# jewettaij/visfd

Measured on AMD Instinct MI355X. Metric: Mvoxels/s (Gauss+DoG+TV pipeline) on 1024^3 float32; % HBM roofline, higher is better.
Workload: dtype f32

## Files before the change

visfd_amd/build.py:

```python
import concurrent.futures
import os
import subprocess
import sys
import time

HERE = os.path.dirname(os.path.abspath(__file__))
ROOT = os.path.dirname(HERE)
CSRC = os.path.join(HERE, "csrc")
OBJDIR = os.path.join(ROOT, "build", "visfd_hip")
LIB = os.path.join(HERE, "libvisfd_hip.so")

SOURCES = ["host_math.cpp", "blob_post.cpp", "connect.cpp", "watershed_host.cpp", "context.hip", "api.hip", "blob_job.hip", "gauss.hip", "blob.hip", "select.hip", "tv.hip", "resample.hip", "slab.hip", "morph.hip", "morph_levels.hip", "extrema.hip", "filter3d.hip", "draw.hip", "watershed.hip", "median.hip", "intensity.hip", "distance.hip", "find_spheres.hip", "discard_overlap.hip", "connect_seeds.hip", "connect_graph_host.cpp", "connect_graph.hip", "voxelize.hip", "surface_points.hip", "close_surface.hip"]
TV_VARIANT = [("tv_tiled.hip", "tv_tiled", ["-fno-slp-vectorize"]), ("tv_box.hip", "tv_box", ["-fno-slp-vectorize"]),
              ("tv_list.hip", "tv_list", ["-fno-slp-vectorize"]),
              ("ridge.hip", "ridge", [])]
PAIR_FLAGS = ["-fno-slp-vectorize"]
VARIANTS = TV_VARIANT + [("gauss_pair.hip", "gauss_pair", PAIR_FLAGS)] + [("gauss_fused.hip", "gauss_fused_h%d" % h, ["-DVH_FUSED_H=%d" % h, "-fno-slp-vectorize"])
                         for h in range(1, 9)]
HEADERS = ["common.hpp", "exact_div.hpp", "tv_common.hpp", "select_pick.hpp", "eigen3.hpp", "union_find.hpp", "tile.hpp", "watershed_host.hpp", "intensity.hpp", "connect_host.hpp", "connect_graph.hpp", os.path.join("..", "..", "include", "visfd_hip.h")]

HIPCC = os.environ.get("HIPCC", "/opt/rocm/bin/hipcc")
FLAGS = ["--offload-arch=gfx950", "-O3", "-std=c++17", "-fPIC", "-ffp-contract=off", "-fno-fast-math",
         "-Wall", "-Wno-unused-function"]


def _mtime(p):
    return os.path.getmtime(p) if os.path.exists(p) else 0.0


def _compile(src, obj, extra=()):
    t0 = time.time()
    cmd = [HIPCC] + FLAGS + list(extra) + ["-x", "hip", "-c", os.path.join(CSRC, src), "-o", obj]
    r = subprocess.run(cmd, capture_output=True, text=True)
    return src, r.returncode, r.stdout + r.stderr, time.time() - t0


def build(force=False, jobs=4, verbose=True):
    os.makedirs(OBJDIR, exist_ok=True)
    newest_header = max(_mtime(os.path.join(CSRC, h)) for h in HEADERS)
    todo, objs = [], []
    units = [(s, os.path.splitext(s)[0], []) for s in SOURCES] + VARIANTS
    flagfile = os.path.join(OBJDIR, "flags.txt")
    flagsig = repr((FLAGS, VARIANTS))
    if not os.path.exists(flagfile) or open(flagfile).read() != flagsig:
        force = True
    for s, stem, extra in units:
        obj = os.path.join(OBJDIR, stem + ".o")
        objs.append(obj)
        if force or _mtime(obj) < max(_mtime(os.path.join(CSRC, s)), newest_header):
            todo.append((s, obj, extra))
    if todo:
        with concurrent.futures.ThreadPoolExecutor(max_workers=jobs) as ex:
            for (src, rc, out, dt), (_, obj, _e) in zip(ex.map(lambda a: _compile(*a), todo), todo):
                if verbose:
                    print("[visfd_amd.build] %-22s %5.1fs %s" % (os.path.basename(obj), dt, "ok" if rc == 0 else "FAILED"))
                if rc != 0:
                    sys.stderr.write(out)
                    raise RuntimeError("hipcc failed on " + src)
                elif out.strip() and verbose:
                    sys.stderr.write(out)
    with open(flagfile, "w") as f:
        f.write(flagsig)
    if todo or not os.path.exists(LIB) or _mtime(LIB) < max(_mtime(o) for o in objs):
        cmd = [HIPCC, "--offload-arch=gfx950", "-shared", "-fPIC", "-o", LIB] + objs
        r = subprocess.run(cmd, capture_output=True, text=True)
        if r.returncode != 0:
            sys.stderr.write(r.stdout + r.stderr)
            raise RuntimeError("link failed")
        if verbose:
            print("[visfd_amd.build] linked", LIB)
    build_cli(verbose)
    return LIB
# ... 28 lines not shown
```

visfd_amd/csrc/api.hip:

```cpp
#include <algorithm>
#include <cmath>
#include <vector>

#include "common.hpp"
#include "tv_common.hpp"

namespace vh {

int gauss_dev(visfd_hip_ctx* ctx, const float* src, float* dst, const float* mask, i64 nx, i64 ny, i64 nz,
              const float sigma[3], const int hw[3], bool normalize, const GaussOpts& o) {
  VH_REQUIRE(ctx && src && dst && sigma && hw, "null argument");
  std::vector<float> t[3];
  for (int d = 0; d < 3; d++) {
    VH_REQUIRE(sigma[d] >= 0.0f, "sigma must be non-negative");
    VH_REQUIRE(hw[d] >= 0 && hw[d] <= MAX_HALFWIDTH, "filter halfwidth must be in [0, 64]");
    t[d].resize(2 * hw[d] + 1);
    host_gauss_taps(sigma[d], hw[d], t[d].data());
  }
  return dev_separable3d(ctx, src, dst, mask, nx, ny, nz, t[0].data(), hw[0], t[1].data(), hw[1], t[2].data(), hw[2],
                         normalize, o);
}

static int log_pair_try(visfd_hip_ctx* ctx, const float* src, float* dst, i64 nx, i64 ny, i64 nz, const float sa[3],
                        const float sb[3], const int hw[3], float scale, float* A, float* B) {
// ... 520 lines not shown
                             float cutoff, int curves) {
  VH_REQUIRE(ctx && sal && dir && ten, "null argument");
  VH_HIP(hipSetDevice(ctx->device));
  VH_TRY(check_dims(nx, ny, nz));
  const Stage st = {ctx, (size_t)(nx * ny * nz)};
  float *dsal, *pdir, *pten, *aos6, *dms = nullptr, *dmd = nullptr;
  VH_TRY(st.up(WS_H2D_0, sal, &dsal));
  VH_TRY(st.up_planar(WS_H2D_1, WS_H2D_2, dir, 3, &pdir));
  VH_TRY(st.out(WS_H2D_3, &pten, 6));
  VH_TRY(st.up(WS_H2D_4, mask_src, &dms));
  if (mask_dst == mask_src) dmd = dms;
  else VH_TRY(st.up(WS_A, mask_dst, &dmd));
  VH_TRY(dev_tv_dense_stick(ctx, dsal, pdir, pten, dms, dmd, nx, ny, nz, 0, nz, sigma_tv, exponent, cutoff, curves != 0));
  VH_TRY(st.out(WS_B, &aos6, 6));
  return st.down_interleaved(ten, pten, aos6, 6, dmd, true);
}

int visfd_hip_tv_weight_sum(visfd_hip_ctx* ctx, const float* sal, float* den, const float* mask_src,
                            const float* mask_dst, int64_t nx, int64_t ny, int64_t nz, float sigma_tv, float cutoff) {
  VH_REQUIRE(ctx && sal && den, "null argument");
  VH_HIP(hipSetDevice(ctx->device));
  VH_TRY(check_dims(nx, ny, nz));
  const Stage st = {ctx, (size_t)(nx * ny * nz)};
  float *dsal, *dden, *dms = nullptr, *dmd = nullptr;
  VH_TRY(st.up(WS_H2D_0, sal, &dsal));
  VH_TRY(st.up(WS_H2D_1, den, &dden));
  VH_TRY(st.up(WS_H2D_4, mask_src, &dms));
  if (mask_dst == mask_src) dmd = dms;
  else VH_TRY(st.up(WS_A, mask_dst, &dmd));
  VH_TRY(dev_tv_weight_sum(ctx, dsal, dden, dms, dmd, nx, ny, nz, sigma_tv, cutoff));
  return st.down(den, dden);
}

static int membrane_queued(visfd_hip_ctx* ctx, i64 nx, i64 ny, i64 nz, float sigma, int order, float best_fraction, float sigma_tv,
                           int exponent, float cutoff, const float* smoothed, float* sal, float* ten, float* dir, bool zero_dir,
                           const float* peak_img, const float* peak_bg, float* thr_out) {
  hipStream_t st = ctx->stream;
  const i64 n = nx * ny * nz;
  VH_TRY(select_rank_check((uint64_t)n, best_fraction));
  if (!ctx->stage_pinned) VH_HIP(hipHostMalloc(&ctx->stage_pinned, sizeof(StageReadback)));
  if (!ctx->stage_event) VH_HIP(hipEventCreateWithFlags(&ctx->stage_event, hipEventDisableTiming));
  StageReadback* block = nullptr;
  VH_TRY(ws(ctx, WS_SELECT, 1, &block));
  VH_HIP(hipMemsetAsync(block, 0, sizeof(*block), st));
  VH_TRY(dev_select_queue(ctx, sal, nullptr, n, best_fraction, &block->sel));
  const float* const thr_dev = &block->sel.thr;
  TvStagePlan plan;
  VH_TRY(dev_tv_stage_count(ctx, sal, thr_dev, nullptr, nx, ny, nz, sigma_tv, exponent, cutoff, &block->list_total,
                            &block->list_flags, &plan));
  const StageReadback* const got = static_cast<const StageReadback*>(ctx->stage_pinned);
  VH_HIP(hipMemcpyAsync(ctx->stage_pinned, block, sizeof(*block), hipMemcpyDeviceToHost, st));
  VH_HIP(hipEventRecord(ctx->stage_event, st));
  if (zero_dir) VH_HIP(hipMemsetAsync(dir, 0, sizeof(float) * 3 * (size_t)n, st));
  VH_TRY(dev_ridge_directions(ctx, smoothed, sal, nx, ny, nz, sigma, order, dir, thr_dev));
  VH_HIP(hipEventSynchronize(ctx->stage_event));
  float thr = 0.0f;
  VH_TRY(select_result(got->sel, &thr));
  if (thr_out) *thr_out = thr;
  int rc = dev_tv_stage_vote(ctx, plan, got->list_total, got->list_flags, sal, dir, ten, nullptr, nx, ny, nz, exponent);
  if (rc == TV_DECLINED) {
    VH_TRY(dev_apply_threshold(ctx, sal, n, thr));
    rc = dev_tv_dense_stick(ctx, sal, dir, ten, nullptr, nullptr, nx, ny, nz, 0, nz, sigma_tv, exponent, cutoff, false);
  }
  VH_TRY(rc);
  return dev_tensor_saliency(ctx, ten, nullptr, n, order, sal, peak_img, peak_bg);
}

static int membrane_stage(visfd_hip_ctx* ctx, const float* src, const float* mask, i64 nx, i64 ny, i64 nz, float sigma, float ratio,
                          int order, float best_fraction, float threshold_abs, float sigma_tv, int exponent, float cutoff,
                          float sigma_background, int normalize_background, float* bg, float* smoothed, float* sal, float* ten,
                          float* dir, bool zero_dir, float* thr_out) {
  const i64 n = nx * ny * nz;
  if (sigma_background > 0.0f)
    VH_TRY(visfd_hip_peak_background_dev(ctx, src, mask, nx, ny, nz, sigma_background, ratio, normalize_background, bg));
  else bg = nullptr;
  VH_TRY(visfd_hip_ridge_scores_bg_dev(ctx, src, mask, nx, ny, nz, sigma, ratio, order, bg, sal, smoothed));
  if (ctx->opt.membrane_queue && sigma_tv > 0.0f && best_fraction >= 0.0f && !mask) {
    const int rc = membrane_queued(ctx, nx, ny, nz, sigma, order, best_fraction, sigma_tv, exponent, cutoff, smoothed, sal, ten, dir,
                                   zero_dir, bg ? src : nullptr, bg, thr_out);
    if (rc != TV_DECLINED) return rc;
  }
  float thr = threshold_abs;
  if (best_fraction >= 0.0f) VH_TRY(dev_threshold_fraction(ctx, sal, mask, n, best_fraction, &thr));
  else VH_TRY(dev_apply_threshold(ctx, sal, n, thr));
  if (thr_out) *thr_out = thr;
  if (zero_dir) VH_HIP(hipMemsetAsync(dir, 0, sizeof(float) * 3 * (size_t)n, ctx->stream));
  VH_TRY(dev_ridge_directions(ctx, smoothed, sal, nx, ny, nz, sigma, order, dir));
  if (sigma_tv > 0.0f) {
    VH_TRY(dev_tv_dense_stick(ctx, sal, dir, ten, mask, mask, nx, ny, nz, 0, nz, sigma_tv, exponent, cutoff, false));
    VH_TRY(dev_tensor_saliency(ctx, ten, mask, n, order, sal, bg ? src : nullptr, bg));
  }
  return VISFD_HIP_OK;
}

int visfd_hip_membrane_detect_bg_dev(visfd_hip_ctx* ctx, const float* src, const float* mask, int64_t nx,
                                     int64_t ny, int64_t nz, float sigma, float ratio, int order,
                                     float best_fraction, float threshold_abs, float sigma_tv, int exponent,
                                     float cutoff, float sigma_background, int normalize_background, float* sal, float* ten,
                                     float* dir, float* thr_out) {
  VH_REQUIRE(ctx && src && sal, "null argument");
  VH_REQUIRE(order == 0 || order == 1, "unsupported eigenvalue order");
  VH_REQUIRE(best_fraction <= 1.0f, "fraction must be <= 1");
  VH_HIP(hipSetDevice(ctx->device));
  VH_TRY(check_dims(nx, ny, nz));
  const i64 n = nx * ny * nz;
  float* d = dir;
  if (!d) VH_TRY(ws(ctx, WS_TVAUX, (size_t)(3 * n), &d));
  float *smoothed = nullptr, *bg = nullptr, *t = ten;
  VH_TRY(ws(ctx, WS_D, (size_t)n, &smoothed));
  if (sigma_background > 0.0f) VH_TRY(ws(ctx, WS_C, (size_t)n, &bg));
  if (!t && sigma_tv > 0.0f) VH_TRY(ws(ctx, WS_B, (size_t)(6 * n), &t));
  return membrane_stage(ctx, src, mask, nx, ny, nz, sigma, ratio, order, best_fraction, threshold_abs, sigma_tv, exponent, cutoff,
                        sigma_background, normalize_background, bg, smoothed, sal, t, d, dir != nullptr, thr_out);
// ... 242 lines not shown
```

visfd_amd/csrc/common.hpp:

```cpp
#pragma once

#include <hip/hip_runtime.h>

#include <cstdint>
#include <cstdio>
#include <cstring>
#include <string>
#include <vector>

#include "../../include/visfd_hip.h"

namespace vh {

typedef int64_t i64;

void set_error(const std::string& msg);
int fail(int code, const std::string& msg);

#define VH_HIP(expr)                                                                         \
  do {                                                                                       \
    hipError_t _e = (expr);                                                                  \
    if (_e != hipSuccess)                                                                    \
      return vh::fail(_e == hipErrorOutOfMemory ? VISFD_HIP_ENOMEM : VISFD_HIP_EDEVICE,      \
                      std::string(#expr) + ": " + hipGetErrorString(_e));                    \
// ... 35 lines not shown
  WS_F3D_TAB,
  WS_DRAW_OWNER,
  WS_DRAW_TAB,
  WS_WSH_KIND,
  WS_WSH_LINK,
  WS_WSH_C,
  WS_WSH_STATE,
  WS_WSH_SEEDS,
  WS_WSH_FLAGS,
  WS_MEDIAN_TAB,
  WS_INTENSITY,
  WS_DIST_DSQ,
  WS_DIST_STACK,
  WS_DIST_POINTS,
  WS_FS_RECORDS,
  WS_FS_QUERIES,
  WS_CG_WORD,
  WS_CG_AUX,
  WS_CG_LIST,
  WS_CG_REC,
  WS_CG_SEEDS,
  WS_CG_CLUSTER,
  WS_CG_COUNTERS,
  WS_CG_SETTLE,
  WS_CG_LINKS,
  WS_OVL_LIST,
  WS_OVL_CELLS,
  WS_OVL_TEMP,
  WS_VOX_TOGGLE,
  WS_VOX_MESH,
  WS_SP_BITS,
  WS_SP_CHUNKS,
  WS_SP_LIST,
  WS_SP_OUT,
  WS_SP_SCRATCH,
  WS_CS_ACC,
  WS_CS_GRID,
  WS_CS_AUX,
  WS_SELECT,
  WS_NSLOTS
};

struct BlobJob;

}

struct visfd_hip_options {
  int gauss_3pass = 0;
  int gauss_cfg = 0;
  int gauss_wg_per_cu = 2;
  int log_pair = 1;
  int log_pair_chunk = 0;
  int membrane_queue = 1;
  int tv_dense = 0;
  int tv_fma = 0;
  int gauss_fma = 0;
  int eig_f32 = 0;
  int tv_zrun = 0;
  int tv_no_replay = 0;
  int tv_exact_tiled = 0;
  int tv_no_fold = 0;
  int tv_poison = 0;
  int tv_reserve_wg = 0;
  int tv_max_wg = 0;
  int64_t blob_test_cap = 0;
  int morph_general = 0;
  int morph_levels = 1;
  int filter3d_general = 0;
  int median_general = 0;
  int distance_general = 0;
  int discard_overlap_host = 0;
  int discard_overlap_time = 0;
  int discard_overlap_max_rounds = 256;
  int find_spheres_host = 0;
  int watershed_host = 0;
  int stats_blocks = 0;
  int connect_time = 0;
  int connect_settle = 0;
  int draw_time = 0;
  int voxelize_bisect = 0;
  int voxelize_time = 0;
  int surface_steps_cap = 256;
  int surface_points_time = 0;
  int close_surface_rtol_exp = 5;
  int close_surface_max_cycles = 20;
  int close_surface_time = 0;
  int debug = 0;
};

struct visfd_hip_ctx {
  visfd_hip_options opt;
  int device = 0;
  hipStream_t stream = nullptr;
  bool own_stream = false;
  void* slot_ptr[vh::WS_NSLOTS] = {};
  size_t slot_bytes[vh::WS_NSLOTS] = {};
  std::vector<unsigned char> slot_key[vh::WS_NSLOTS];
  int num_cus = 256;
  hipStream_t aux_stream = nullptr;
  void* stage_pinned = nullptr;
  hipEvent_t stage_event = nullptr;
  int morph_last_path = -1;
  struct {
    int64_t n = 0, ncols = 0;
    float den = 0.0f;
  } f3d;
// ... 360 lines not shown
```

visfd_amd/csrc/context.hip:

```cpp
#include <cctype>
#include <cstdlib>

#include "common.hpp"

namespace vh {

static thread_local std::string g_last_error;
void set_error(const std::string& msg) { g_last_error = msg; }
int fail(int code, const std::string& msg) {
  g_last_error = msg;
  return code;
}

int ws_get(visfd_hip_ctx* ctx, Slot s, size_t bytes, void** out) {
  if (bytes == 0) bytes = 16;
  if (ctx->slot_bytes[s] < bytes) {
    ctx->slot_key[s].clear();
    if (ctx->slot_ptr[s] && (s == WS_CAND || s == WS_SCANCNT)) VH_TRY(blob_jobs_drain(ctx));
    if (ctx->slot_ptr[s]) {
      VH_HIP(hipStreamSynchronize(ctx->stream));
      VH_HIP(hipFree(ctx->slot_ptr[s]));
      ctx->slot_ptr[s] = nullptr;
      ctx->slot_bytes[s] = 0;
    }
    void* p = nullptr;
    hipError_t e = hipMalloc(&p, bytes);
    if (e != hipSuccess)
      return fail(VISFD_HIP_ENOMEM, "hipMalloc of " + std::to_string(bytes) + " bytes failed: " +
                                        hipGetErrorString(e));
    ctx->slot_ptr[s] = p;
    ctx->slot_bytes[s] = bytes;
  }
  *out = ctx->slot_ptr[s];
  return VISFD_HIP_OK;
}

bool ws_holds(const visfd_hip_ctx* ctx, Slot s, const void* key, size_t key_bytes) {
  const std::vector<unsigned char>& k = ctx->slot_key[s];
  return key_bytes > 0 && k.size() == key_bytes && std::memcmp(k.data(), key, key_bytes) == 0;
}

int ws_put(visfd_hip_ctx* ctx, Slot s, const void* key, size_t key_bytes, const void* host, size_t bytes) {
  ctx->slot_key[s].clear();
  VH_HIP(hipStreamSynchronize(ctx->stream));
  void* d = nullptr;
  VH_TRY(ws_get(ctx, s, bytes, &d));
  VH_HIP(hipMemcpyAsync(d, host, bytes, hipMemcpyHostToDevice, ctx->stream));
  VH_HIP(hipStreamSynchronize(ctx->stream));
  const unsigned char* k = static_cast<const unsigned char*>(key);
  ctx->slot_key[s].assign(k, k + key_bytes);
  return VISFD_HIP_OK;
}

namespace {

struct OptionDesc {
  const char* name;
  int visfd_hip_options::*i = nullptr;
  int64_t visfd_hip_options::*l = nullptr;
  OptionDesc(const char* n, int visfd_hip_options::*f) : name(n), i(f) {}
  OptionDesc(const char* n, int64_t visfd_hip_options::*f) : name(n), l(f) {}
};
#define VH_OPT(field) {#field, &visfd_hip_options::field}
const OptionDesc kOptions[] = {
    VH_OPT(gauss_3pass), VH_OPT(gauss_cfg), VH_OPT(gauss_wg_per_cu), VH_OPT(log_pair), VH_OPT(log_pair_chunk),
    VH_OPT(membrane_queue),
    VH_OPT(tv_dense), VH_OPT(tv_fma), VH_OPT(gauss_fma), VH_OPT(eig_f32), VH_OPT(tv_zrun), VH_OPT(tv_no_replay),
    VH_OPT(tv_exact_tiled), VH_OPT(tv_no_fold), VH_OPT(tv_poison), VH_OPT(tv_reserve_wg), VH_OPT(tv_max_wg),
    VH_OPT(blob_test_cap), VH_OPT(morph_general), VH_OPT(morph_levels), VH_OPT(filter3d_general), VH_OPT(median_general),
    VH_OPT(distance_general), VH_OPT(discard_overlap_host), VH_OPT(discard_overlap_time),
    VH_OPT(discard_overlap_max_rounds), VH_OPT(find_spheres_host), VH_OPT(watershed_host), VH_OPT(stats_blocks),
    VH_OPT(connect_time), VH_OPT(connect_settle), VH_OPT(draw_time), VH_OPT(voxelize_bisect), VH_OPT(voxelize_time),
    VH_OPT(surface_steps_cap), VH_OPT(surface_points_time), VH_OPT(close_surface_rtol_exp),
    VH_OPT(close_surface_max_cycles), VH_OPT(close_surface_time), VH_OPT(debug),
};
#undef VH_OPT
bool set_option(visfd_hip_options* o, const char* name, int64_t value) {
  for (const OptionDesc& d : kOptions) {
    if (std::strcmp(d.name, name) != 0) continue;
    if (d.i) o->*(d.i) = (int)value; else o->*(d.l) = value;
    return true;
  }
  return false;
}
bool get_option(const visfd_hip_options* o, const char* name, int64_t* value) {
  for (const OptionDesc& d : kOptions) {
    if (std::strcmp(d.name, name) != 0) continue;
    *value = d.i ? (int64_t)(o->*(d.i)) : o->*(d.l);
    return true;
  }
  return false;
}
void options_from_environment(visfd_hip_options* o) {
  for (const OptionDesc& d : kOptions) {
    std::string env = "VISFD_HIP_";
    for (const char* c = d.name; *c; c++) env += (char)std::toupper((unsigned char)*c);
    if (const char* e = std::getenv(env.c_str())) set_option(o, d.name, (int64_t)std::atoll(e));
  }
}

}
}

using namespace vh;

extern "C" {

int visfd_hip_abi_version(void) { return 10; }
const char* visfd_hip_last_error(void) { return g_last_error.c_str(); }

int visfd_hip_create(int device, void* stream, visfd_hip_ctx** out) {
  VH_REQUIRE(out, "null output pointer");
  int count = 0;
  hipError_t e = hipGetDeviceCount(&count);
  if (e != hipSuccess || count <= 0)
    return fail(VISFD_HIP_EDEVICE, "no HIP device available (libvisfd_hip has no CPU fallback)");
  VH_REQUIRE(device >= 0 && device < count, "bad device ordinal");
  VH_HIP(hipSetDevice(device));
  hipDeviceProp_t prop;
// ... 91 lines not shown
```

visfd_amd/csrc/ridge.hip:

```cpp
#include "common.hpp"
#include "eigen3.hpp"

namespace vh {

namespace {

constexpr int BLOCK = 256;

struct Stencil {
  const float* S;
  i64 c;
  i64 sx, sy, sz;
  __device__ __forceinline__ float at(int dx, int dy, int dz) const {
    return S[c + dx * sx + dy * sy + dz * sz];
  }
};

__device__ __forceinline__ void hessian_at(const Stencil& f, float s2, float h6[6]) {
  const float f0 = f.at(0, 0, 0);
  const float two_f0 = 2 * f0;
  const float hxx = (f.at(1, 0, 0) + f.at(-1, 0, 0)) - two_f0;
  const float hyy = (f.at(0, 1, 0) + f.at(0, -1, 0)) - two_f0;
  const float hzz = (f.at(0, 0, 1) + f.at(0, 0, -1)) - two_f0;
  const float hxy = 0.25f * (((f.at(1, 1, 0) + f.at(-1, -1, 0)) - f.at(1, -1, 0)) - f.at(-1, 1, 0));
  const float hyz = 0.25f * (((f.at(0, 1, 1) + f.at(0, -1, -1)) - f.at(0, 1, -1)) - f.at(0, -1, 1));
  const float hzx = 0.25f * (((f.at(1, 0, 1) + f.at(-1, 0, -1)) - f.at(-1, 0, 1)) - f.at(1, 0, -1));
  h6[0] = hxx * s2; h6[1] = hyy * s2; h6[2] = hzz * s2;
  h6[3] = hxy * s2; h6[4] = hyz * s2; h6[5] = hzx * s2;
}

__device__ __forceinline__ bool voxel_of_block(int nx, int ny, int& ix, int& iy, int& iz) {
  const int xblocks = (nx + BLOCK - 1) / BLOCK;
  unsigned b = blockIdx.x;
  const int bx = b % xblocks;
  b /= xblocks;
  iy = b % ny;
  iz = b / ny;
  ix = bx * BLOCK + threadIdx.x;
  return ix < nx;
}

__device__ __forceinline__ Stencil clamped_stencil(const float* S, int ix, int iy, int iz, int nx, int ny,
                                                   int nz) {
  const int x = min(max(ix, 1), nx - 2), y = min(max(iy, 1), ny - 2), z = min(max(iz, 1), nz - 2);
  Stencil f;
  f.S = S;
  f.sx = 1; f.sy = nx; f.sz = (i64)nx * ny;
  f.c = (i64)z * f.sz + (i64)y * nx + x;
  return f;
}

template <bool F32>
__device__ __forceinline__ void saliency_dir(const float h6[6], int order, float& sal, float dir[3]) {
  float d6[6];
  eig::diagonalize_flat<F32>(h6, order, d6);
  const double l1 = d6[0], l2 = d6[1];
  double N = l1 * l1 - l2 * l2;
  N *= N;
  sal = (float)N;
  eig::shoemake_row0(d6 + 3, dir);
}

__global__ void __launch_bounds__(BLOCK)
hessian_kernel(const float* __restrict__ S, const float* __restrict__ mask, int nx, int ny, int nz,
               float sigma, float* __restrict__ grad, float* __restrict__ hess) {
  int ix, iy, iz;
  if (!voxel_of_block(nx, ny, ix, iy, iz)) return;
  const i64 nvox = (i64)nx * ny * nz;
  const i64 v = ((i64)iz * ny + iy) * nx + ix;
  if (mask && mask[v] == 0.0f) return;
  const Stencil f = clamped_stencil(S, ix, iy, iz, nx, ny, nz);
  if (grad) {
    const float g0 = 0.5f * (f.at(1, 0, 0) - f.at(-1, 0, 0));
    const float g1 = 0.5f * (f.at(0, 1, 0) - f.at(0, -1, 0));
    const float g2 = 0.5f * (f.at(0, 0, 1) - f.at(0, 0, -1));
    grad[v] = g0 * sigma;
    grad[nvox + v] = g1 * sigma;
    grad[2 * nvox + v] = g2 * sigma;
  }
  if (hess) {
    float h6[6];
    hessian_at(f, sigma * sigma, h6);
#pragma unroll
    for (int c = 0; c < 6; c++) hess[c * nvox + v] = h6[c];
  }
}

template <bool F32>
__global__ void __launch_bounds__(BLOCK)
hessian_saliency_kernel(const float* __restrict__ hess, const float* __restrict__ mask, i64 nvox,
                        int order, float* __restrict__ sal, float* __restrict__ dir) {
  const i64 v = (i64)blockIdx.x * BLOCK + threadIdx.x;
  if (v >= nvox) return;
  if (mask && mask[v] == 0.0f) { sal[v] = 0.0f; return; }
  float h6[6];
#pragma unroll
  for (int c = 0; c < 6; c++) h6[c] = hess[c * nvox + v];
  float s, d[3];
  saliency_dir<F32>(h6, order, s, d);
  sal[v] = s;
  dir[v] = d[0];
  dir[nvox + v] = d[1];
  dir[2 * nvox + v] = d[2];
}

template <bool F32>
__global__ void __launch_bounds__(BLOCK)
ridge_fused_kernel(const float* __restrict__ S, const float* __restrict__ mask, int nx, int ny, int nz,
                   float sigma, int order, float* __restrict__ sal, float* __restrict__ dir) {
  int ix, iy, iz;
  if (!voxel_of_block(nx, ny, ix, iy, iz)) return;
  const i64 nvox = (i64)nx * ny * nz;
  const i64 v = ((i64)iz * ny + iy) * nx + ix;
// ... 263 lines not shown
```

visfd_amd/csrc/tv_common.hpp:

```cpp
#pragma once

#include <algorithm>

#include "common.hpp"

namespace vh {

constexpr int TV_DECLINED = -1;

inline int tv_padded_row(int h) {
  int sp = 2 * h + 1;
  while ((sp & 7) != 4) sp++;
  return sp;
}

inline int tv_box_row(int h) {
  int sp = 2 * h + 1 + 3;
  while ((sp & 7) != 4) sp++;
  return sp;
}
inline int tv_box_slice(int h) { return (2 * h + 1 + 6) * tv_box_row(h) + 8; }

struct TvTableLayout {
  size_t packed, padded, box_tol, box_exact, box_tol_sq;
// ... 31 lines not shown

inline int tv_plan_units(const visfd_hip_ctx* ctx, int default_zrun, int tiles_x, int tiles_y, i64 z_out0, i64 z_out1,
                         int* zrun, i64* nblk) {
  int zr = default_zrun;
  if (ctx->opt.tv_zrun >= 1 && ctx->opt.tv_zrun <= 4096) zr = ctx->opt.tv_zrun;
  if ((i64)zr > z_out1 - z_out0) zr = (int)(z_out1 - z_out0);
  if (zr < 1) zr = 1;
  const i64 nruns = (z_out1 - z_out0 + zr - 1) / zr;
  *zrun = zr;
  *nblk = std::max<i64>((i64)tiles_x * tiles_y * nruns, 0);
  if (*nblk > 0x7fffffffLL) return fail(VISFD_HIP_EINVAL, "volume too large for one launch");
  return VISFD_HIP_OK;
}
inline i64 tv_plan_grid(const visfd_hip_ctx* ctx, size_t wg_per_cu, i64 nblk) {
  i64 ngrid = (i64)ctx->num_cus * (i64)wg_per_cu;
  if (ctx->opt.tv_reserve_wg > 0) ngrid = std::max<i64>(ngrid - ctx->opt.tv_reserve_wg, 1);
  if (ctx->opt.tv_max_wg > 0 && ngrid > ctx->opt.tv_max_wg) ngrid = ctx->opt.tv_max_wg;
  return std::min(ngrid, nblk);
}

template <typename... KArgs, typename... Args>
inline int tv_launch_lds(visfd_hip_ctx* ctx, void (*kernel)(KArgs...), i64 ngrid, int nthreads, size_t lds, Args... args) {
  VH_HIP(hipFuncSetAttribute(reinterpret_cast<const void*>(kernel), hipFuncAttributeMaxDynamicSharedMemorySize, (int)lds));
  kernel<<<dim3((unsigned)ngrid), dim3(nthreads), lds, ctx->stream>>>(args...);
  return VISFD_HIP_OK;
}

int dev_tv_tiled(visfd_hip_ctx* ctx, const float* sal, const float* dir, float* ten, const float* mask_src,
                 const float* mask_dst, i64 nx, i64 ny, i64 nz, i64 z_out0, i64 z_out1, int h, const float4* dtab, int exponent,
                 bool curves, bool weights_only);
int dev_tv_box(visfd_hip_ctx* ctx, const float* sal, const float* dir, float* ten, const float* mask_src, const float* mask_dst,
               i64 nx, i64 ny, i64 nz, i64 z_out0, i64 z_out1, int h, const float4* dtab_box, const float4* dtab_box_sq, int exponent,
               bool exact);


constexpr int TV_LIST_MAX_NX = 16384;
constexpr unsigned TVL_NOT_POSITIVE = 1u;
constexpr unsigned TVL_NON_FINITE = 2u;
constexpr unsigned TVL_WEIGHTED_MASK = 4u;
struct TvSenderLists {
  const float4* ent;
  const unsigned* pos;
  const unsigned* rows;
  unsigned long long total;
  unsigned flags;
  bool folded;
  int zl0, nzl;
};
struct TvListGeo {
  int nx, ny, nz;
  int zl0, nzl;
  int ntx, h;
};
struct TvListPlan {
  TvListGeo g;
  unsigned* rows;
  unsigned row_blocks;
  int mode;
  const float* thr_dev;
};
int tv_list_count(visfd_hip_ctx* ctx, const float* sal, const float* thr_dev, const float* mask_src, i64 nx, i64 ny, i64 nz,
                  i64 z_out0, i64 z_out1, int h, int mode, unsigned* counter, unsigned long long* total_dev, unsigned* flags_dev,
                  TvListPlan* plan);
int tv_list_write(visfd_hip_ctx* ctx, const TvListPlan& plan, const float* sal, const float* dir, const float* mask_src,
                  unsigned long long total, unsigned flags, unsigned decline_on, bool may_fold, TvSenderLists* out);

int dev_tv_box_count(visfd_hip_ctx* ctx, const float* sal, const float* thr_dev, const float* mask_src, i64 nx, i64 ny, i64 nz,
                     i64 z_out0, i64 z_out1, int h, int exponent, bool exact, unsigned long long* total_dev, unsigned* flags_dev,
                     TvListPlan* plan);
int dev_tv_box_vote(visfd_hip_ctx* ctx, const TvListPlan& plan, unsigned long long total, unsigned flags, const float* sal,
                    const float* dir, float* ten, const float* mask_src, const float* mask_dst, i64 nx, i64 ny, i64 nz, i64 z_out0,
                    i64 z_out1, int h, const float4* dtab_box, const float4* dtab_box_sq, int exponent, bool exact);

struct TvStagePlan {
  int h;
  bool exact;
  const float4 *dtab_box, *dtab_box_sq;
  TvListPlan lists;
};
int dev_tv_stage_count(visfd_hip_ctx* ctx, const float* sal, const float* thr_dev, const float* mask, i64 nx, i64 ny, i64 nz,
                       float sigma_tv, int exponent, float cutoff, unsigned long long* total_dev, unsigned* flags_dev,
                       TvStagePlan* plan);
int dev_tv_stage_vote(visfd_hip_ctx* ctx, const TvStagePlan& plan, unsigned long long total, unsigned flags, const float* sal,
                      const float* dir, float* ten, const float* mask, i64 nx, i64 ny, i64 nz, int exponent);

}
```

visfd_amd/csrc/tv_list.hip:

```cpp
#include <algorithm>

#include "tv_common.hpp"

namespace vh {

using namespace box_tile;

namespace {

using ListGeo = TvListGeo;
constexpr int LNT = 256;
constexpr int LWORDS_MAX = TV_LIST_MAX_NX / 32;

__device__ __forceinline__ unsigned popc_range(const unsigned* w, int lo, int hi) {
  unsigned c = 0;
  for (int i = lo >> 5; i <= (hi - 1) >> 5 && lo < hi; i++) {
    unsigned m = w[i];
    if (i == (lo >> 5)) m &= ~0u << (lo & 31);
    if (i == ((hi - 1) >> 5) && (hi & 31)) m &= ~0u >> (32 - (hi & 31));
    c += (unsigned)__builtin_popcount(m);
  }
  return c;
}

template <bool WRITE, int MODE>
__global__ void __launch_bounds__(LNT)
tvl_row_kernel(const float* __restrict__ sal, const float* __restrict__ dir, const float* __restrict__ mask_src, ListGeo g,
               unsigned* __restrict__ rows, float4* __restrict__ ent, unsigned* __restrict__ pos,
               unsigned* __restrict__ neg_flag ,
               int fold ,
               const float* __restrict__ thr_dev ) {
  constexpr int LB = 8;
  __shared__ unsigned bits_all[LNT / 64][LWORDS_MAX + 4];
  __shared__ unsigned base_all[WRITE ? LNT / 64 : 1][WRITE ? LWORDS_MAX * 2 + 4 : 1];
  __shared__ unsigned cum_all[WRITE ? LNT / 64 : 1][WRITE ? LWORDS_MAX / 2 + 4 : 1];
  const int wave = __builtin_amdgcn_readfirstlane((int)threadIdx.x >> 6), lane = threadIdx.x & 63;
  const i64 r = (i64)blockIdx.x * (LNT / 64) + wave;
  if (r >= (i64)g.nzl * g.ny) return;
  unsigned* const bits = bits_all[wave];
  const int y = (int)(r % g.ny), zl = (int)(r / g.ny);
  const i64 plane = (i64)g.nx * g.ny, nvox = plane * g.nz;
  const i64 row = (i64)(g.zl0 + zl) * plane + (i64)y * g.nx;
  const int nchunks = (g.nx + 63) >> 6;
  unsigned* const rrow = rows + ((size_t)zl * (size_t)(g.ny + 1) + (size_t)y) * (size_t)g.ntx;
  if (WRITE) {
    unsigned* const base = base_all[WRITE ? wave : 0];
    for (int tx = lane; tx < g.ntx; tx += 64) base[tx] = rrow[g.ntx + tx];
  }
  unsigned any = 0, total = 0;
  unsigned* const cum = cum_all[WRITE ? wave : 0];
  const bool cut = thr_dev != nullptr;
  const float thr = cut ? *thr_dev : 0.0f;
  for (int c0 = 0; c0 < nchunks; c0 += LB) {
    float v[LB], m[LB];
// ... 21 lines not shown
        if (!(__builtin_fabsf(s) <= 3.402823466e38f)) atomicOr(neg_flag, 2u);
        if (mask_src && m[k] != 1.0f) atomicOr(neg_flag, 4u);
      }
    }
  }
  __builtin_amdgcn_wave_barrier();
  asm volatile("s_waitcnt vmcnt(0) lgkmcnt(0)" ::: "memory");
  if (!WRITE) {
    for (int tx = lane; tx < g.ntx; tx += 64)
      rrow[tx] = any ? popc_range(bits, max(TX * tx - g.h, 0), min(TX * tx + TX + g.h, g.nx)) : 0u;
    return;
  }
  if (!any) return;
  const unsigned* const base = base_all[WRITE ? wave : 0];
  for (unsigned j0 = 0; j0 < total; j0 += 64) {
    const unsigned j = j0 + lane;
    if (j >= total) break;
    int lo = 0, hi = nchunks;
    while (hi - lo > 1) {
      const int mid = (lo + hi) >> 1;
      if (cum[mid] <= j) lo = mid; else hi = mid;
    }
    unsigned k = j - cum[lo];
    unsigned w = bits[2 * lo];
    int x = 64 * lo;
    {
      const unsigned t = (unsigned)__builtin_popcount(w);
      if (k >= t) { k -= t; x += 32; w = bits[2 * lo + 1]; }
    }
#pragma unroll
    for (int sft = 16; sft >= 1; sft >>= 1) {
      const unsigned t = (unsigned)__builtin_popcount(w & ((1u << sft) - 1u));
      if (k >= t) { k -= t; x += sft; w >>= sft; }
    }
    float4 q = make_float4(sal[row + x] * (MODE == 0 ? 0.25f : (MODE == 2 ? 0.5f : 1.0f)), dir[row + x], dir[nvox + row + x], dir[2 * nvox + row + x]);
    if (mask_src) q.x = q.x * mask_src[row + x];
    if (fold) {
      const double r2 = sqrt((double)q.x);
      const float a = (float)(MODE == 0 ? cbrt(r2) : sqrt(r2));
      q = make_float4(2.0f * a * a, a * q.y, a * q.z, a * q.w);
    }
    const int t0 = max((x - TX - g.h) / TX + ((x - TX - g.h) >= 0 ? 1 : 0), 0);
    const int t1 = min((x + g.h) / TX, g.ntx - 1);
    for (int tx = t0; tx <= t1; tx++) {
      const int lo_x = TX * tx - g.h, hi_x = min(TX * tx + TX + g.h, g.nx);
      if (x < lo_x || x >= hi_x) continue;
      const unsigned idx = base[tx] + popc_range(bits, x + 1, hi_x);
      ent[idx] = q;
      pos[idx] = (unsigned)(x - lo_x) | ((unsigned)y << 8);
    }
  }
}

__global__ void __launch_bounds__(LNT)
tvl_scan_kernel(ListGeo g, unsigned* __restrict__ rows, unsigned long long* __restrict__ total) {
  const int i = blockIdx.x * LNT + threadIdx.x;
  if (i >= g.nzl * g.ntx) return;
  const int zl = i / g.ntx, tx = i - zl * g.ntx;
  unsigned* const col = rows + (size_t)zl * (size_t)(g.ny + 1) * (size_t)g.ntx + tx;
  unsigned sum = 0;
  for (int y = 0; y < g.ny; y++) sum += col[(size_t)y * g.ntx];
  const unsigned base = (unsigned)atomicAdd(total, (unsigned long long)sum);
  unsigned run = base;
  unsigned prev = col[(size_t)(g.ny - 1) * g.ntx];
  col[(size_t)g.ny * g.ntx] = run;
  for (int y = g.ny - 1; y >= 0; y--) {
    const unsigned c = prev;
    if (y > 0) prev = col[(size_t)(y - 1) * g.ntx];
    run += c;
    col[(size_t)y * g.ntx] = run;
  }
}

}

namespace {
auto row_kernel(bool write, int mode) {
  if (write) return mode == 1 ? tvl_row_kernel<true, 1> : mode == 0 ? tvl_row_kernel<true, 0> : tvl_row_kernel<true, 2>;
  return mode == 1 ? tvl_row_kernel<false, 1> : mode == 0 ? tvl_row_kernel<false, 0> : tvl_row_kernel<false, 2>;
}
}

int tv_list_count(visfd_hip_ctx* ctx, const float* sal, const float* thr_dev, const float* mask_src, i64 nx, i64 ny, i64 nz,
                  i64 z_out0, i64 z_out1, int h, int mode, unsigned* counter, unsigned long long* total_dev, unsigned* flags_dev,
                  TvListPlan* plan) {
  hipStream_t st = ctx->stream;
  ListGeo g;
  g.nx = (int)nx; g.ny = (int)ny; g.nz = (int)nz; g.h = h; g.ntx = (int)((nx + TX - 1) / TX);
  g.zl0 = (int)std::max<i64>(z_out0 - h, 0);
  g.nzl = (int)(std::min<i64>(z_out1 + h, nz) - g.zl0);
  const size_t nrows = (size_t)g.nzl * (size_t)(ny + 1) * (size_t)g.ntx;
  if ((i64)g.nzl * ny > 0x7fffffffLL) return TV_DECLINED;
  unsigned* rows = nullptr;
  if (ws(ctx, WS_TVLIST, nrows, &rows) != VISFD_HIP_OK) { set_error(""); (void)hipGetLastError(); return TV_DECLINED; }
  VH_HIP(hipMemsetAsync(counter, 0, 16 * sizeof(unsigned), st));
  const unsigned row_blocks = (unsigned)(((i64)g.nzl * ny + LNT / 64 - 1) / (LNT / 64));
  row_kernel(false, mode)<<<dim3(row_blocks), dim3(LNT), 0, st>>>(sal, nullptr, mask_src, g, rows, nullptr, nullptr, flags_dev, 0, thr_dev);
  tvl_scan_kernel<<<dim3((unsigned)(((size_t)g.nzl * g.ntx + LNT - 1) / LNT)), dim3(LNT), 0, st>>>(g, rows, total_dev);
  VH_HIP(hipGetLastError());
  *plan = {g, rows, row_blocks, mode, thr_dev};
  return VISFD_HIP_OK;
}

int tv_list_write(visfd_hip_ctx* ctx, const TvListPlan& plan, const float* sal, const float* dir, const float* mask_src,
                  unsigned long long total, unsigned flags, unsigned decline_on, bool may_fold, TvSenderLists* out) {
  hipStream_t st = ctx->stream;
  if (flags & decline_on) return TV_DECLINED;
  if (total >= (1ull << 32) - 2048) return TV_DECLINED;
  const int fold = (may_fold && !(flags & TVL_NOT_POSITIVE)) ? 1 : 0;
  unsigned char* lists = nullptr;
  if (ws(ctx, WS_TVSCRATCH, (size_t)(total + 16) * 20, &lists) != VISFD_HIP_OK) { set_error(""); (void)hipGetLastError(); return TV_DECLINED; }
  float4* const ent = reinterpret_cast<float4*>(lists);
  unsigned* const pos = reinterpret_cast<unsigned*>(lists + (size_t)(total + 16) * 16);
  if (ctx->opt.tv_poison) VH_HIP(hipMemsetAsync(lists, 0xff, (size_t)(total + 16) * 20, st));
  row_kernel(true, plan.mode)<<<dim3(plan.row_blocks), dim3(LNT), 0, st>>>(sal, dir, mask_src, plan.g, plan.rows, ent, pos, nullptr, fold,
                                                                           plan.thr_dev);
  VH_HIP(hipGetLastError());
  *out = {ent, pos, plan.rows, total, flags, fold != 0, plan.g.zl0, plan.g.nzl};
  return VISFD_HIP_OK;
}

}
```

Before: 2700.

## Fuse ridge direction computation into the tensor-voting list sender pass

Instead of running a dense ridge-direction kernel over every voxel before voting, the list-write pass now computes the Hessian, eigen-decomposition and direction only for voxels that pass the saliency threshold, writing dir and the sender entries in one kernel. It aims to remove the dense eigen solve and a full read/write pass over the volume. On decline, the dense ridge pass is run afterwards as a fallback. The fused path adds stencil gathers inside a compaction loop and only applies to whole unmasked volumes.

Result: no change. 2704, median of 3 (+0.2%).

```diff
diff --git a/visfd_amd/build.py b/visfd_amd/build.py
--- a/visfd_amd/build.py
+++ b/visfd_amd/build.py
@@ -17,7 +17,7 @@
 PAIR_FLAGS = ["-fno-slp-vectorize"]
 VARIANTS = TV_VARIANT + [("gauss_pair.hip", "gauss_pair", PAIR_FLAGS)] + [("gauss_fused.hip", "gauss_fused_h%d" % h, ["-DVH_FUSED_H=%d" % h, "-fno-slp-vectorize"])
                          for h in range(1, 9)]
-HEADERS = ["common.hpp", "exact_div.hpp", "tv_common.hpp", "select_pick.hpp", "eigen3.hpp", "union_find.hpp", "tile.hpp", "watershed_host.hpp", "intensity.hpp", "connect_host.hpp", "connect_graph.hpp", os.path.join("..", "..", "include", "visfd_hip.h")]
+HEADERS = ["common.hpp", "exact_div.hpp", "tv_common.hpp", "select_pick.hpp", "eigen3.hpp", "ridge_dev.hpp", "union_find.hpp", "tile.hpp", "watershed_host.hpp", "intensity.hpp", "connect_host.hpp", "connect_graph.hpp", os.path.join("..", "..", "include", "visfd_hip.h")]
 
 HIPCC = os.environ.get("HIPCC", "/opt/rocm/bin/hipcc")
 FLAGS = ["--offload-arch=gfx950", "-O3", "-std=c++17", "-fPIC", "-ffp-contract=off", "-fno-fast-math",
diff --git a/visfd_amd/csrc/api.hip b/visfd_amd/csrc/api.hip
--- a/visfd_amd/csrc/api.hip
+++ b/visfd_amd/csrc/api.hip
@@ -596,13 +596,16 @@
   VH_HIP(hipMemcpyAsync(ctx->stage_pinned, block, sizeof(*block), hipMemcpyDeviceToHost, st));
   VH_HIP(hipEventRecord(ctx->stage_event, st));
   if (zero_dir) VH_HIP(hipMemsetAsync(dir, 0, sizeof(float) * 3 * (size_t)n, st));
-  VH_TRY(dev_ridge_directions(ctx, smoothed, sal, nx, ny, nz, sigma, order, dir, thr_dev));
+  const bool fuse = ctx->opt.membrane_fuse != 0;
+  if (fuse) plan.lists.ridge = {smoothed, dir, sigma, order};
+  else VH_TRY(dev_ridge_directions(ctx, smoothed, sal, nx, ny, nz, sigma, order, dir, thr_dev));
   VH_HIP(hipEventSynchronize(ctx->stage_event));
   float thr = 0.0f;
   VH_TRY(select_result(got->sel, &thr));
   if (thr_out) *thr_out = thr;
   int rc = dev_tv_stage_vote(ctx, plan, got->list_total, got->list_flags, sal, dir, ten, nullptr, nx, ny, nz, exponent);
   if (rc == TV_DECLINED) {
+    if (fuse) VH_TRY(dev_ridge_directions(ctx, smoothed, sal, nx, ny, nz, sigma, order, dir, thr_dev));
     VH_TRY(dev_apply_threshold(ctx, sal, n, thr));
     rc = dev_tv_dense_stick(ctx, sal, dir, ten, nullptr, nullptr, nx, ny, nz, 0, nz, sigma_tv, exponent, cutoff, false);
   }
diff --git a/visfd_amd/csrc/common.hpp b/visfd_amd/csrc/common.hpp
--- a/visfd_amd/csrc/common.hpp
+++ b/visfd_amd/csrc/common.hpp
@@ -111,6 +111,7 @@
   int log_pair = 1;
   int log_pair_chunk = 0;
   int membrane_queue = 1;
+  int membrane_fuse = 1;
   int tv_dense = 0;
   int tv_fma = 0;
   int gauss_fma = 0;
diff --git a/visfd_amd/csrc/context.hip b/visfd_amd/csrc/context.hip
--- a/visfd_amd/csrc/context.hip
+++ b/visfd_amd/csrc/context.hip
@@ -64,7 +64,7 @@
 #define VH_OPT(field) {#field, &visfd_hip_options::field}
 const OptionDesc kOptions[] = {
     VH_OPT(gauss_3pass), VH_OPT(gauss_cfg), VH_OPT(gauss_wg_per_cu), VH_OPT(log_pair), VH_OPT(log_pair_chunk),
-    VH_OPT(membrane_queue),
+    VH_OPT(membrane_queue), VH_OPT(membrane_fuse),
     VH_OPT(tv_dense), VH_OPT(tv_fma), VH_OPT(gauss_fma), VH_OPT(eig_f32), VH_OPT(tv_zrun), VH_OPT(tv_no_replay),
     VH_OPT(tv_exact_tiled), VH_OPT(tv_no_fold), VH_OPT(tv_poison), VH_OPT(tv_reserve_wg), VH_OPT(tv_max_wg),
     VH_OPT(blob_test_cap), VH_OPT(morph_general), VH_OPT(morph_levels), VH_OPT(filter3d_general), VH_OPT(median_general),
diff --git a/visfd_amd/csrc/ridge.hip b/visfd_amd/csrc/ridge.hip
--- a/visfd_amd/csrc/ridge.hip
+++ b/visfd_amd/csrc/ridge.hip
@@ -1,5 +1,6 @@
 #include "common.hpp"
 #include "eigen3.hpp"
+#include "ridge_dev.hpp"
 
 namespace vh {
 
@@ -7,27 +8,10 @@
 
 constexpr int BLOCK = 256;
 
-struct Stencil {
-  const float* S;
-  i64 c;
-  i64 sx, sy, sz;
-  __device__ __forceinline__ float at(int dx, int dy, int dz) const {
-    return S[c + dx * sx + dy * sy + dz * sz];
-  }
-};
-
-__device__ __forceinline__ void hessian_at(const Stencil& f, float s2, float h6[6]) {
-  const float f0 = f.at(0, 0, 0);
-  const float two_f0 = 2 * f0;
-  const float hxx = (f.at(1, 0, 0) + f.at(-1, 0, 0)) - two_f0;
-  const float hyy = (f.at(0, 1, 0) + f.at(0, -1, 0)) - two_f0;
-  const float hzz = (f.at(0, 0, 1) + f.at(0, 0, -1)) - two_f0;
-  const float hxy = 0.25f * (((f.at(1, 1, 0) + f.at(-1, -1, 0)) - f.at(1, -1, 0)) - f.at(-1, 1, 0));
-  const float hyz = 0.25f * (((f.at(0, 1, 1) + f.at(0, -1, -1)) - f.at(0, 1, -1)) - f.at(0, -1, 1));
-  const float hzx = 0.25f * (((f.at(1, 0, 1) + f.at(-1, 0, -1)) - f.at(-1, 0, 1)) - f.at(1, 0, -1));
-  h6[0] = hxx * s2; h6[1] = hyy * s2; h6[2] = hzz * s2;
-  h6[3] = hxy * s2; h6[4] = hyz * s2; h6[5] = hzx * s2;
-}
+using ridge_dev::Stencil;
+using ridge_dev::clamped_stencil;
+using ridge_dev::hessian_at;
+using ridge_dev::saliency_dir;
 
 __device__ __forceinline__ bool voxel_of_block(int nx, int ny, int& ix, int& iy, int& iz) {
   const int xblocks = (nx + BLOCK - 1) / BLOCK;
@@ -38,27 +22,6 @@
   iz = b / ny;
   ix = bx * BLOCK + threadIdx.x;
   return ix < nx;
-}
-
-__device__ __forceinline__ Stencil clamped_stencil(const float* S, int ix, int iy, int iz, int nx, int ny,
-                                                   int nz) {
-  const int x = min(max(ix, 1), nx - 2), y = min(max(iy, 1), ny - 2), z = min(max(iz, 1), nz - 2);
-  Stencil f;
-  f.S = S;
-  f.sx = 1; f.sy = nx; f.sz = (i64)nx * ny;
-  f.c = (i64)z * f.sz + (i64)y * nx + x;
-  return f;
-}
-
-template <bool F32>
-__device__ __forceinline__ void saliency_dir(const float h6[6], int order, float& sal, float dir[3]) {
-  float d6[6];
-  eig::diagonalize_flat<F32>(h6, order, d6);
-  const double l1 = d6[0], l2 = d6[1];
-  double N = l1 * l1 - l2 * l2;
-  N *= N;
-  sal = (float)N;
-  eig::shoemake_row0(d6 + 3, dir);
 }
 
 __global__ void __launch_bounds__(BLOCK)
diff --git a/visfd_amd/csrc/ridge_dev.hpp b/visfd_amd/csrc/ridge_dev.hpp
--- /dev/null
+++ b/visfd_amd/csrc/ridge_dev.hpp
@@ -0,0 +1,52 @@
+#pragma once
+#include "common.hpp"
+#include "eigen3.hpp"
+
+namespace vh {
+namespace ridge_dev {
+
+struct Stencil {
+  const float* S;
+  i64 c;
+  i64 sx, sy, sz;
+  __device__ __forceinline__ float at(int dx, int dy, int dz) const {
+    return S[c + dx * sx + dy * sy + dz * sz];
+  }
+};
+
+__device__ __forceinline__ void hessian_at(const Stencil& f, float s2, float h6[6]) {
+  const float f0 = f.at(0, 0, 0);
+  const float two_f0 = 2 * f0;
+  const float hxx = (f.at(1, 0, 0) + f.at(-1, 0, 0)) - two_f0;
+  const float hyy = (f.at(0, 1, 0) + f.at(0, -1, 0)) - two_f0;
+  const float hzz = (f.at(0, 0, 1) + f.at(0, 0, -1)) - two_f0;
+  const float hxy = 0.25f * (((f.at(1, 1, 0) + f.at(-1, -1, 0)) - f.at(1, -1, 0)) - f.at(-1, 1, 0));
+  const float hyz = 0.25f * (((f.at(0, 1, 1) + f.at(0, -1, -1)) - f.at(0, 1, -1)) - f.at(0, -1, 1));
+  const float hzx = 0.25f * (((f.at(1, 0, 1) + f.at(-1, 0, -1)) - f.at(-1, 0, 1)) - f.at(1, 0, -1));
+  h6[0] = hxx * s2; h6[1] = hyy * s2; h6[2] = hzz * s2;
+  h6[3] = hxy * s2; h6[4] = hyz * s2; h6[5] = hzx * s2;
+}
+
+__device__ __forceinline__ Stencil clamped_stencil(const float* S, int ix, int iy, int iz, int nx, int ny,
+                                                   int nz) {
+  const int x = min(max(ix, 1), nx - 2), y = min(max(iy, 1), ny - 2), z = min(max(iz, 1), nz - 2);
+  Stencil f;
+  f.S = S;
+  f.sx = 1; f.sy = nx; f.sz = (i64)nx * ny;
+  f.c = (i64)z * f.sz + (i64)y * nx + x;
+  return f;
+}
+
+template <bool F32>
+__device__ __forceinline__ void saliency_dir(const float h6[6], int order, float& sal, float dir[3]) {
+  float d6[6];
+  eig::diagonalize_flat<F32>(h6, order, d6);
+  const double l1 = d6[0], l2 = d6[1];
+  double N = l1 * l1 - l2 * l2;
+  N *= N;
+  sal = (float)N;
+  eig::shoemake_row0(d6 + 3, dir);
+}
+
+}
+}
diff --git a/visfd_amd/csrc/tv_common.hpp b/visfd_amd/csrc/tv_common.hpp
--- a/visfd_amd/csrc/tv_common.hpp
+++ b/visfd_amd/csrc/tv_common.hpp
@@ -107,12 +107,19 @@
   int zl0, nzl;
   int ntx, h;
 };
+struct TvListRidge {
+  const float* smoothed = nullptr;
+  float* dir = nullptr;
+  float sigma = 0.0f;
+  int order = 0;
+};
 struct TvListPlan {
   TvListGeo g;
   unsigned* rows;
   unsigned row_blocks;
   int mode;
   const float* thr_dev;
+  TvListRidge ridge = {};
 };
 int tv_list_count(visfd_hip_ctx* ctx, const float* sal, const float* thr_dev, const float* mask_src, i64 nx, i64 ny, i64 nz,
                   i64 z_out0, i64 z_out1, int h, int mode, unsigned* counter, unsigned long long* total_dev, unsigned* flags_dev,
diff --git a/visfd_amd/csrc/tv_list.hip b/visfd_amd/csrc/tv_list.hip
--- a/visfd_amd/csrc/tv_list.hip
+++ b/visfd_amd/csrc/tv_list.hip
@@ -1,5 +1,6 @@
 #include <algorithm>
 
+#include "ridge_dev.hpp"
 #include "tv_common.hpp"
 
 namespace vh {
@@ -127,6 +128,101 @@
   }
 }
 
+template <int MODE, bool F32>
+__global__ void __launch_bounds__(LNT, 4)
+tvl_send_kernel(const float* __restrict__ sal, const float* __restrict__ S , ListGeo g,
+                const unsigned* __restrict__ rows, float4* __restrict__ ent, unsigned* __restrict__ pos, int fold,
+                const float* __restrict__ thr_dev, float* __restrict__ dir, float sigma, int order) {
+  constexpr int LB = 8;
+  __shared__ unsigned bits_all[LNT / 64][LWORDS_MAX + 4];
+  __shared__ unsigned base_all[LNT / 64][LWORDS_MAX * 2 + 4];
+  __shared__ unsigned cum_all[LNT / 64][LWORDS_MAX / 2 + 4];
+  const int wave = __builtin_amdgcn_readfirstlane((int)threadIdx.x >> 6), lane = threadIdx.x & 63;
+  const i64 r = (i64)blockIdx.x * (LNT / 64) + wave;
+  if (r >= (i64)g.nzl * g.ny) return;
+  unsigned* const bits = bits_all[wave];
+  unsigned* const base = base_all[wave];
+  unsigned* const cum = cum_all[wave];
+  const int y = (int)(r % g.ny), zl = (int)(r / g.ny);
+  const i64 plane = (i64)g.nx * g.ny, nvox = plane * g.nz;
+  const i64 row = (i64)(g.zl0 + zl) * plane + (i64)y * g.nx;
+  const int nchunks = (g.nx + 63) >> 6;
+  const unsigned* const rrow = rows + ((size_t)zl * (size_t)(g.ny + 1) + (size_t)y) * (size_t)g.ntx;
+  for (int tx = lane; tx < g.ntx; tx += 64) base[tx] = rrow[g.ntx + tx];
+  unsigned any = 0, total = 0;
+  const bool cut = thr_dev != nullptr;
+  const float thr = cut ? *thr_dev : 0.0f;
+  for (int c0 = 0; c0 < nchunks; c0 += LB) {
+    float v[LB];
+#pragma unroll
+    for (int k = 0; k < LB; k++) {
+      const int x = 64 * (c0 + k) + lane;
+      v[k] = x < g.nx ? sal[row + x] : 0.0f;
+    }
+#pragma unroll
+    for (int k = 0; k < LB; k++) {
+      if (c0 + k >= nchunks) break;
+      const bool f = v[k] != 0.0f && !(cut && v[k] < thr);
+      const unsigned long long bal = __builtin_amdgcn_ballot_w64(f);
+      if (lane == 0) {
+        bits[2 * (c0 + k)] = (unsigned)bal;
+        bits[2 * (c0 + k) + 1] = (unsigned)(bal >> 32);
+        cum[c0 + k] = total;
+      }
+      any |= (unsigned)bal | (unsigned)(bal >> 32);
+      total += (unsigned)__builtin_popcountll(bal);
+    }
+  }
+  __builtin_amdgcn_wave_barrier();
+  asm volatile("s_waitcnt vmcnt(0) lgkmcnt(0)" ::: "memory");
+  if (!any) return;
+  const float s2 = sigma * sigma;
+  for (unsigned j0 = 0; j0 < total; j0 += 64) {
+    const unsigned j = j0 + lane;
+    if (j >= total) break;
+    int lo = 0, hi = nchunks;
+    while (hi - lo > 1) {
+      const int mid = (lo + hi) >> 1;
+      if (cum[mid] <= j) lo = mid; else hi = mid;
+    }
+    unsigned k = j - cum[lo];
+    unsigned w = bits[2 * lo];
+    int x = 64 * lo;
+    {
+      const unsigned t = (unsigned)__builtin_popcount(w);
+      if (k >= t) { k -= t; x += 32; w = bits[2 * lo + 1]; }
+    }
+#pragma unroll
+    for (int sft = 16; sft >= 1; sft >>= 1) {
+      const unsigned t = (unsigned)__builtin_popcount(w & ((1u << sft) - 1u));
+      if (k >= t) { k -= t; x += sft; w >>= sft; }
+    }
+    const float sv = sal[row + x];
+    const ridge_dev::Stencil f = ridge_dev::clamped_stencil(S, x, y, g.zl0 + zl, g.nx, g.ny, g.nz);
+    float h6[6], s, d[3];
+    ridge_dev::hessian_at(f, s2, h6);
+    ridge_dev::saliency_dir<F32>(h6, order, s, d);
+    dir[row + x] = d[0];
+    dir[nvox + row + x] = d[1];
+    dir[2 * nvox + row + x] = d[2];
+    float4 q = make_float4(sv * (MODE == 0 ? 0.25f : (MODE == 2 ? 0.5f : 1.0f)), d[0], d[1], d[2]);
+    if (fold) {
+      const double r2 = sqrt((double)q.x);
+      const float a = (float)(MODE == 0 ? cbrt(r2) : sqrt(r2));
+      q = make_float4(2.0f * a * a, a * q.y, a * q.z, a * q.w);
+    }
+    const int t0 = max((x - TX - g.h) / TX + ((x - TX - g.h) >= 0 ? 1 : 0), 0);
+    const int t1 = min((x + g.h) / TX, g.ntx - 1);
+    for (int tx = t0; tx <= t1; tx++) {
+      const int lo_x = TX * tx - g.h, hi_x = min(TX * tx + TX + g.h, g.nx);
+      if (x < lo_x || x >= hi_x) continue;
+      const unsigned idx = base[tx] + popc_range(bits, x + 1, hi_x);
+      ent[idx] = q;
+      pos[idx] = (unsigned)(x - lo_x) | ((unsigned)y << 8);
+    }
+  }
+}
+
 __global__ void __launch_bounds__(LNT)
 tvl_scan_kernel(ListGeo g, unsigned* __restrict__ rows, unsigned long long* __restrict__ total) {
   const int i = blockIdx.x * LNT + threadIdx.x;
@@ -154,6 +250,8 @@
   if (write) return mode == 1 ? tvl_row_kernel<true, 1> : mode == 0 ? tvl_row_kernel<true, 0> : tvl_row_kernel<true, 2>;
   return mode == 1 ? tvl_row_kernel<false, 1> : mode == 0 ? tvl_row_kernel<false, 0> : tvl_row_kernel<false, 2>;
 }
+template <bool F32>
+auto send_kernel(int mode) { return mode == 1 ? tvl_send_kernel<1, F32> : mode == 0 ? tvl_send_kernel<0, F32> : tvl_send_kernel<2, F32>; }
 }
 
 int tv_list_count(visfd_hip_ctx* ctx, const float* sal, const float* thr_dev, const float* mask_src, i64 nx, i64 ny, i64 nz,
@@ -188,8 +286,15 @@
   float4* const ent = reinterpret_cast<float4*>(lists);
   unsigned* const pos = reinterpret_cast<unsigned*>(lists + (size_t)(total + 16) * 16);
   if (ctx->opt.tv_poison) VH_HIP(hipMemsetAsync(lists, 0xff, (size_t)(total + 16) * 20, st));
-  row_kernel(true, plan.mode)<<<dim3(plan.row_blocks), dim3(LNT), 0, st>>>(sal, dir, mask_src, plan.g, plan.rows, ent, pos, nullptr, fold,
-                                                                           plan.thr_dev);
+  if (const TvListRidge& r = plan.ridge; r.smoothed) {
+    if (mask_src || plan.g.zl0 != 0 || plan.g.nzl != plan.g.nz) return fail(VISFD_HIP_EINVAL, "the sender pass takes whole unmasked volumes");
+    auto kernel = ctx->opt.eig_f32 ? send_kernel<true>(plan.mode) : send_kernel<false>(plan.mode);
+    kernel<<<dim3(plan.row_blocks), dim3(LNT), 0, st>>>(sal, r.smoothed, plan.g, plan.rows, ent, pos, fold, plan.thr_dev, r.dir, r.sigma,
+                                                        r.order);
+  } else {
+    row_kernel(true, plan.mode)<<<dim3(plan.row_blocks), dim3(LNT), 0, st>>>(sal, dir, mask_src, plan.g, plan.rows, ent, pos, nullptr, fold,
+                                                                             plan.thr_dev);
+  }
   VH_HIP(hipGetLastError());
   *out = {ent, pos, plan.rows, total, flags, fold != 0, plan.g.zl0, plan.g.nzl};
   return VISFD_HIP_OK;
```
